# SeunghwanByun/SLAM-RGBD

Measured on AMD Instinct MI355X. Metric: ICP frame-pair aligns/sec @640×480 (1/2/4/8 GPU); SE(3) err vs CPU ref, higher is better.
Workload: dtype fp32

## Files before the change

### slam-rgbd_amd/csrc/icp_api.cpp

```cpp

#include <stdio.h>
#include <stdlib.h>
#include <string.h>

#include <algorithm>
#include <cmath>
#include <vector>

#include "icp_host.h"

using namespace youth_icp;

namespace youth_icp {

thread_local youth::ErrorText g_icp_err;

hipStream_t pick_stream(youth_icp_ctx* c, void* stream)
{
    return stream ? (hipStream_t)stream : c->stream;
}

int bind_device(youth_icp_ctx* c)
{
    HIP_TRY(hipSetDevice(c->device));
// ... 187 lines not shown
        return fail("hipMalloc depth", e);
    if ((e = hipMalloc(&c->d_rec, rec_bytes)) != hipSuccess) return fail("hipMalloc rec", e);
    if ((e = hipMemset(c->d_rec, 0, rec_bytes)) != hipSuccess) return fail("memset rec", e);
    if ((e = hipMalloc(&c->d_T64, MF * 16 * sizeof(double))) != hipSuccess)
        return fail("hipMalloc T64", e);
    if ((e = hipMalloc(&c->d_T32, MF * 12 * sizeof(float))) != hipSuccess)
        return fail("hipMalloc T32", e);
    if ((e = hipMalloc(&c->d_status, MF * sizeof(int32_t))) != hipSuccess)
        return fail("hipMalloc status", e);
    if ((e = hipMalloc(&c->d_Tinit, MF * 16 * sizeof(double))) != hipSuccess)
        return fail("hipMalloc Tinit", e);
    if ((e = hipMalloc(&c->d_neq, MF * kNeq * sizeof(double))) != hipSuccess)
        return fail("hipMalloc neq", e);
    if ((e = hipMalloc(&c->d_Tout, MF * 16 * sizeof(float))) != hipSuccess)
        return fail("hipMalloc Tout", e);
    if ((e = hipMalloc(&c->d_flag, 16)) != hipSuccess) return fail("hipMalloc flag", e);
    if ((e = hipMalloc(&c->d_epoch, MF * sizeof(unsigned))) != hipSuccess)
        return fail("hipMalloc epoch", e);
    if ((e = hipMalloc(&c->d_head, kQWords * 4)) != hipSuccess) return fail("hipMalloc head", e);
    if ((e = hipMemset(c->d_head, 0, kQWords * 4)) != hipSuccess) return fail("memset head", e);
    {
        hipDeviceProp_t prop;
        if ((e = hipGetDeviceProperties(&prop, device)) != hipSuccess)
            return fail("hipGetDeviceProperties", e);
        c->n_cu = prop.multiProcessorCount;
        const char* what = nullptr;
        if ((e = fill_occupancy(c, &what)) != hipSuccess) return fail(what, e);
        const char* np = getenv("YOUTH_ICP_NO_PERSISTENT");
        c->persistent = !(np && *np && *np != '0');
        const char* nif = getenv("YOUTH_ICP_NO_IDENT_FIRST");
        c->ident_first = ident_first_ok(Kd) && !(nif && *nif && *nif != '0');
        const char* ifm = getenv("YOUTH_ICP_IDENT_FIRST");
        c->ident_prep = !(ifm && strcmp(ifm, "icp") == 0);
        const char* pst = getenv("YOUTH_ICP_PREP_STRIP");
        if (pst && atoi(pst) >= 1) c->prep_strip = atoi(pst);
        const char* cth = getenv("YOUTH_ICP_COOP_THREADS");
        if (cth && atoi(cth) == 256) c->coop_threads = 256;
        const char* nc = getenv("YOUTH_ICP_NO_COOP");
        c->coop = !(nc && *nc && *nc != '0');
        const char* cpd = getenv("YOUTH_ICP_COOP_POLL_DELAY");
        if (cpd && atoi(cpd) >= 0) c->coop_poll_delay = atoi(cpd);
        const char* cpx = getenv("YOUTH_ICP_COOP_PX");
        if (cpx && atoi(cpx) >= 1 && atoi(cpx) <= kCoopMaxPx) c->coop_px = atoi(cpx);
        c->coop_px_env = c->coop_px;
        const char* cl = getenv("YOUTH_ICP_COOP_LAUNCH");
        c->coop_launch = !cl ? 0 : strcmp(cl, "runtime") == 0 ? 1 : strcmp(cl, "plain") == 0 ? 2 : 0;
        const char* tcp = getenv("YOUTH_ICP_TRACK_COPY");
        c->trk_copy_compute = tcp && strcmp(tcp, "compute") == 0;
        c->trk_copy_sdma = tcp && (strcmp(tcp, "sdma") == 0 || c->trk_copy_compute);
        const char* pwg = getenv("YOUTH_ICP_PULL_WG");
        c->trk_pull_wg = pwg && atoi(pwg) > 0 ? std::min(atoi(pwg), 1024) : 0;
        const char* plds = getenv("YOUTH_ICP_PULL_LDS");
        if (plds && atoi(plds) >= 0) c->trk_pull_lds = std::min(atoi(plds), 64 << 10);
        const char* pres = getenv("YOUTH_ICP_PULL_RESERVE_CU");
        if (pres && atoi(pres) >= 0) c->trk_pull_reserve = atoi(pres);
        const char* cpt = getenv("YOUTH_ICP_COPY_THREADS");
        if (cpt && atoi(cpt) >= 0) c->trk_copy_helpers = std::min(atoi(cpt), 15);
        const char* cst = getenv("YOUTH_ICP_TEST_COOP_STALL");
        if (cst && atoi(cst) >= 0) {
            c->coop_stall_once = atoi(cst);
            const char* colon = strchr(cst, ':');
            c->coop_stall_left = colon && atoi(colon + 1) > 0 ? atoi(colon + 1) : 1;
            fprintf(stderr, "youth_icp: TEST HOOK YOUTH_ICP_TEST_COOP_STALL=%s active: the first %d "
                            "cooperative launch(es) of this context time out\n",
                    cst, c->coop_stall_left);
        }
        const char* sit = getenv("YOUTH_ICP_TEST_COOP_STALL_ITER");
        if (sit && atoi(sit) >= 0) c->coop_stall_iter = atoi(sit);
// ... 348 lines not shown
```

### slam-rgbd_amd/csrc/icp_device.h

```cpp
#ifndef YOUTH_ICP_DEVICE_H
#define YOUTH_ICP_DEVICE_H

#include <hip/hip_runtime.h>

#include <stdint.h>

#include "youth_icp.h"

namespace {

constexpr int kTileW = 64;
constexpr int kPrepThreads = 512;
#ifndef YOUTH_PREP_TW
#define YOUTH_PREP_TW 128
#endif
#ifndef YOUTH_PREP_TH
#define YOUTH_PREP_TH 24
#endif
constexpr int kPrepTW = YOUTH_PREP_TW;
constexpr int kPrepTH = YOUTH_PREP_TH;
constexpr int kLdsW = kTileW + 2;

constexpr int kRedThreads = 256;
constexpr int kRedStep = kRedThreads * 4;
constexpr int kNeq = YOUTH_NEQ;
constexpr int kPartStride = 30;
constexpr int kPieces = kPartStride / 2;
constexpr int kSumCols = 16;
constexpr int kQHead = 0, kQError = 32, kQSpins = 64, kQWaited = 96, kQHeads = 128;
constexpr int kMaxQueues = 8, kQHeadStride = 32;
constexpr int kQWords = kQHeads + kMaxQueues * kQHeadStride;

typedef float f4v __attribute__((ext_vector_type(4)));
typedef unsigned u4v __attribute__((ext_vector_type(4)));

struct Intr {
    float fx, fy, cx, cy, ds;
};

struct FastK {
    float hfx, lfx, hfy, lfy, hds, lds;
};

__device__ __forceinline__ double join64(unsigned lo, unsigned hi)
{
    return __hiloint2double((int)hi, (int)lo);
}
__device__ __forceinline__ unsigned lo32(double x) { return (unsigned)__double2loint(x); }
__device__ __forceinline__ unsigned hi32(double x) { return (unsigned)__double2hiint(x); }

__device__ __forceinline__ double readlane64(double x, int l)
{
    return join64((unsigned)__builtin_amdgcn_readlane((int)lo32(x), l),
// ... 63 lines not shown
{
    return (len2 >= 0x1p-96f) && (len2 <= 0x1p118f) && norm_comp_ok(cx) && norm_comp_ok(cy) &&
           norm_comp_ok(cz);
}
__device__ __forceinline__ float norm_div(float c, float len, float r)
{
    return copysignf(proj_quot(fabsf(c), len, r), c);
}
__device__ __forceinline__ bool norm_fast_ok_bits(float len2, float cx, float cy, float cz)
{
    constexpr unsigned kLo = 0x0F800000u, kHi = 0x7A800000u, kTiny = 2u * 0x1F800000u - 2u;
    const unsigned tx = (__float_as_uint(cx) << 1) - 2u, ty = (__float_as_uint(cy) << 1) - 2u,
                   tz = (__float_as_uint(cz) << 1) - 2u;
    return (int)((__float_as_uint(len2) - kLo) <= (kHi - kLo)) & (int)(min(min(tx, ty), tz) >= kTiny);
}

template <bool kFast>
__device__ __forceinline__ void backproject(int d, int u, int v, const Intr& K,
                                            const FastK& F, float& x, float& y, float& z)
{
    const float zz = bp_div<kFast>((float)max(d, 0), K.ds, F.hds, F.lds);
    x = bp_div<kFast>(((float)u - K.cx) * zz, K.fx, F.hfx, F.lfx);
    y = bp_div<kFast>(((float)v - K.cy) * zz, K.fy, F.hfy, F.lfy);
    z = zz;
}
template <bool kFast>
__device__ __forceinline__ void backproject_c(int d, float uc, float vc, const Intr& K,
                                              const FastK& F, float& x, float& y, float& z)
{
    const float zz = bp_div<kFast>((float)max(d, 0), K.ds, F.hds, F.lds);
    x = bp_div<kFast>(uc * zz, K.fx, F.hfx, F.lfx);
    y = bp_div<kFast>(vc * zz, K.fy, F.hfy, F.lfy);
    z = zz;
}

__device__ __forceinline__ double dd2(double a, double b, double c, double d)
{
    return fma(a, b, -(c * d));
}
__device__ __forceinline__ double dot3(double a0, double b0, double a1, double b1, double a2,
                                       double b2)
{
    return fma(a2, b2, fma(a1, b1, a0 * b0));
}
__device__ __forceinline__ void adj3(const double* p, double* c)
{
    c[0] = dd2(p[3], p[5], p[4], p[4]);
    c[1] = dd2(p[2], p[4], p[1], p[5]);
    c[2] = dd2(p[1], p[4], p[2], p[3]);
    c[3] = dd2(p[0], p[5], p[2], p[2]);
    c[4] = dd2(p[1], p[2], p[0], p[4]);
    c[5] = dd2(p[0], p[3], p[1], p[1]);
}
__device__ __forceinline__ void symv3(const double* c, const double* v, double* o)
{
    o[0] = dot3(c[0], v[0], c[1], v[1], c[2], v[2]);
    o[1] = dot3(c[1], v[0], c[3], v[1], c[4], v[2]);
    o[2] = dot3(c[2], v[0], c[4], v[1], c[5], v[2]);
}
__device__ __forceinline__ int solve_block6(const double* neq, double xi[6])
{
#pragma unroll
    for (int i = 0; i < 6; ++i) xi[i] = 0.0;
    if (!(neq[28] >= 6.0)) return YOUTH_STATUS_FEW_MATCHES;
    double maxd = 0.0;
    maxd = neq[0] > maxd ? neq[0] : maxd;
// ... 498 lines not shown
```

### slam-rgbd_amd/csrc/icp_host.h

```cpp
#ifndef YOUTH_ICP_HOST_H
#define YOUTH_ICP_HOST_H

#include <hip/hip_runtime.h>

#include <stddef.h>
#include <stdint.h>

#include <memory>
#include <string>
#include <vector>

#include "hip_host.h"
#include "host_copy.h"
#include "icp_device.h"
#include "youth_icp.h"

namespace youth_icp __attribute__((visibility("hidden"))) {

extern thread_local youth::ErrorText g_icp_err;

}

#define HIP_ERR youth_icp::g_icp_err

// ... 9 lines not shown
    int W = 0, H = 0, N = 0;
    size_t P = 0;
    int max_frames = 0;
    Intr K{};
    FastK F{};
    bool fast = false;
    bool centred_exact = true;
    int spec = kSpecSurvey;
    youth_icp_params prm{};
    hipStream_t stream = nullptr;

    int16_t* d_depth = nullptr;
    float4* d_rec = nullptr;
    float* d_xyz = nullptr;
    double* d_T64 = nullptr;
    float* d_T32 = nullptr;
    int32_t* d_status = nullptr;
    double* d_Tinit = nullptr;
    double* d_stats = nullptr;
    int stats_iters = 0;
    double* d_partials = nullptr;
    size_t partials_cap = 0;
    double* d_neq = nullptr;
    int32_t* d_assoc = nullptr;
    float* d_Tout = nullptr;
    unsigned* d_flag = nullptr;
    unsigned* d_arrivals = nullptr;
    unsigned* d_arr_it = nullptr;
    unsigned* d_epoch = nullptr;
    unsigned* d_head = nullptr;
    bool persistent = true;
    bool ident_first = true;
    bool ident_prep = true;
    int prep_strip = 0;
    int last_first_form = 0;
    int reduce = YOUTH_REDUCE_EXACT;
    youth_lanes lanes{};
    bool has_lanes = false;
    bool lanes_mixed = false;
    int icp_blocks_per_cu[4 * kVariants] = {};
    int n_cu = 0;
    bool coop = true;
    int coop_px = 0;
    int coop_px_env = 0;
    int coop_threads = 512;
    int coop_max_pairs = kCoopMaxPairs;
    int coop_launch = 0;
    bool trk_copy_compute = false;
    bool trk_copy_sdma = false;
    int trk_pull_wg = 0;
    int trk_pull_lds = 48 << 10;
    int trk_pull_reserve = 32;
    int trk_copy_helpers = 3;
    size_t trk_copy_min = 1u << 20;
    std::unique_ptr<youth::HostCopyPool> copy_pool;
    bool coop_refuse = false;
    int coop_bpc[2][2 * kVariants][kCoopMaxPx + 1] = {};
    int coop_bpc_tall[2 * kVariants] = {};
    unsigned* d_coop = nullptr;
    int32_t* d_status_out = nullptr;
    int coop_par = 0;
    double* d_coop_part = nullptr;
    int coop_part_cap = 0;
    int coop_part_rows[2] = {0, 0};
    int coop_poll_delay = -1;
    int coop_stall_once = -1;
    int coop_stall_left = 0;
// ... 115 lines not shown
```

### slam-rgbd_amd/csrc/icp_kernels.hip

```cpp

#include <hip/hip_runtime.h>

#include <stdint.h>
#include <stdio.h>
#include <stdlib.h>

#include <algorithm>
#include <cmath>
#include <condition_variable>
#include <mutex>

#include "icp_device.h"
#include "icp_host.h"

namespace {

__global__ void k_verify_fastdiv(Intr K, FastK F, int W, int H, unsigned* bad)
{
    const int d = blockIdx.x * blockDim.x + threadIdx.x + 1;
    if (d > 32767) return;
    const float zi = (float)d / K.ds;
    unsigned nb = (div_fast((float)d, F.hds, F.lds) != zi);
    for (int u = blockIdx.y; u < W; u += gridDim.y) {
        const float n = ((float)u - K.cx) * zi;
// ... 124 lines not shown
    constexpr unsigned kLo = 0x0F800000u, kHi = 0x7A800000u;
    for (unsigned long long b = kLo + tid; b <= kHi; b += stride) {
        const float x = __uint_as_float((unsigned)b);
        b0 += __float_as_uint(sqrt_rn_mid(x)) != __float_as_uint(sqrtf(x));
    }
    for (unsigned long long i = tid; i < n; i += stride) {
        unsigned long long st = seed ^ (i * 0xD1B54A32D192ED03ull);
        const int e0 = (int)(sm64(st) % 131) - 70;
        float c[3];
#pragma unroll
        for (int k = 0; k < 3; ++k) {
            const unsigned long long r = sm64(st);
            const int e = max(e0 - (int)((r >> 32) % 48), -126);
            const unsigned sign = (unsigned)(r >> 63) << 31;
            c[k] = ((r >> 56) & 7) == 0
                       ? __uint_as_float(sign)
                       : __uint_as_float(sign | (unsigned)((e + 127) << 23) |
                                         (unsigned)(r & 0x7FFFFF));
        }
        const float len2 = (c[0] * c[0] + c[1] * c[1]) + c[2] * c[2];
        b1 += norm_fast_ok_bits(len2, c[0], c[1], c[2]) != norm_fast_ok(len2, c[0], c[1], c[2]);
        if (!(len2 > 0.0f) || !norm_fast_ok(len2, c[0], c[1], c[2])) continue;
        ++nf;
        const float len = sqrt_rn_mid(len2), r = proj_recip(len), ref = sqrtf(len2);
#pragma unroll
        for (int k = 0; k < 3; ++k)
            b1 += __float_as_uint(norm_div(c[k], len, r)) != __float_as_uint(c[k] / ref);
    }
    if (b0) atomicAdd(bad + 0, b0);
    if (b1) atomicAdd(bad + 1, b1);
    if (nf) atomicAdd(bad + 2, nf);
}

template <bool kFast, bool kWide, bool kSc1, int kThreads, int kTH, int kTW = kTileW, typename Fn>
__device__ __forceinline__ void prep_tile_with(const int16_t* __restrict__ dep,
                                               float4* __restrict__ R, int W, int H, size_t P,
                                               const Intr& K, const FastK& F,
                                               float* __restrict__ X, int x0, int y0, float* sX,
                                               float* sY, float* sZ, Fn&& per_record)
{
    constexpr int kLH = kTH + 2;
    constexpr int kLW = kTW + 2;
    static_assert(kTW % 64 == 0 && kThreads % kTW == 0, "rows of whole waves");
    static_assert(kTH % (kThreads / kTW) == 0, "tile rows a multiple of the rows per step");
    static_assert(3 * (kTH + 2) * (kTW + 2) * sizeof(float) <= 160 * 1024, "LDS planes fit");
    const int tx = threadIdx.x % kTW;
    const int ty = threadIdx.x / kTW;
    if (kWide) {
        static_assert(2 * kLH <= kThreads, "one edge pixel per thread");
        const bool edge = threadIdx.x < 2 * kLH;
        const int ely = threadIdx.x >> 1, eright = threadIdx.x & 1;
        const int egy = y0 - 1 + ely, egx = eright ? x0 + kTW : x0 - 1;
        const __amdgpu_buffer_rsrc_t rdep = __builtin_amdgcn_make_buffer_rsrc(
            const_cast<int16_t*>(dep), (short)0, W * H * (int)sizeof(int16_t), 0x00020000);
        const bool ein = edge & ((unsigned)egy < (unsigned)H) & ((unsigned)egx < (unsigned)W);
        unsigned short dedge =
            __builtin_amdgcn_raw_buffer_load_b16(rdep, ein ? (egy * W + egx) * 2 : W * H * 2, 0, 0);
        constexpr int kWords = kTW / 4;
        constexpr int kIt = (kLH * kWords + kThreads - 1) / kThreads;
        short4 wd[kIt];
#pragma unroll
        for (int it = 0; it < kIt; ++it) {
            const int e = threadIdx.x + it * kThreads;
            const int ly = e / kWords;
            const int gy = y0 - 1 + ly;
            const int c = x0 + 4 * (e - ly * kWords);
            const bool inside = (e < kLH * kWords) & ((unsigned)gy < (unsigned)H) & (c < W);
            wd[it] = __builtin_bit_cast(
                short4, __builtin_amdgcn_raw_buffer_load_b64(rdep, inside ? (gy * W + c) * 2 : W * H * 2, 0, 0));
        }
#pragma unroll
        for (int it = 0; it < kIt; ++it) {
// ... 39 lines not shown
            const int ly = e / kLW;
            const int lx = e - ly * kLW;
            const int gx = x0 - 1 + lx, gy = y0 - 1 + ly;
            float x = 0.0f, y = 0.0f, z = 0.0f;
            if (gx >= 0 && gx < W && gy >= 0 && gy < H)
                backproject<kFast>(dep[(size_t)gy * W + gx], gx, gy, K, F, x, y, z);
            sX[ly * kLW + lx] = x;
            sY[ly * kLW + lx] = y;
            sZ[ly * kLW + lx] = z;
        }
    }
    __syncthreads();

    const __amdgpu_buffer_rsrc_t rrec =
        __builtin_amdgcn_make_buffer_rsrc(R, (short)0, (int)(P * sizeof(float4)), 0x00020000);
    const int tyw = __builtin_amdgcn_readfirstlane(ty);
#pragma unroll
    for (int k = 0; k < kTH / (kThreads / kTW); ++k) {
        const int row = tyw + (kThreads / kTW) * k;
        const int gx = x0 + tx, gy = y0 + row;
        if (gx >= W || gy >= H) continue;
        const size_t i = (size_t)gy * W + gx;
        const int ly = row + 1, lx = tx + 1;
        const int o = ly * kLW + lx;
        const float px = sX[o], py = sY[o], pz = sZ[o];
        if (X) {
            X[i] = px;
            X[P + i] = py;
            X[2 * P + i] = pz;
        }
        const bool inner = (gx > 0) & (gy > 0) & (gx < W - 1) & (gy < H - 1);
        const float zl = sZ[o - 1], zr = sZ[o + 1];
        const float zu = sZ[o - kLW], zd = sZ[o + kLW];
        const unsigned zmin = min(min(min(__float_as_uint(pz), __float_as_uint(zl)),
                                      min(__float_as_uint(zr), __float_as_uint(zu))),
                                  __float_as_uint(zd));
        const float ax = sX[o + 1] - sX[o - 1];
        const float ay = sY[o + 1] - sY[o - 1];
        const float az = zr - zl;
        const float bx = sX[o + kLW] - sX[o - kLW];
        const float by = sY[o + kLW] - sY[o - kLW];
        const float bz = zd - zu;
        const float cx = ay * bz - az * by;
        const float cy = az * bx - ax * bz;
        const float cz = ax * by - ay * bx;
        const float len2 = (cx * cx + cy * cy) + cz * cz;
        const bool has_n = inner & (zmin != 0u) & (len2 > 0.0f);
        const float len = sqrt_rn_mid(len2);
        const float r = proj_recip(len);
        float nx = norm_div(cx, len, r);
        float ny = norm_div(cy, len, r);
        float nz = norm_div(cz, len, r);
        if (__builtin_expect(has_n & !norm_fast_ok_bits(len2, cx, cy, cz), 0)) {
            const float l = sqrtf(len2);
            nx = cx / l;
            ny = cy / l;
            nz = cz / l;
        }
        if (((nx * px + ny * py) + nz * pz) > 0.0f) {
            nx = -nx;
            ny = -ny;
            nz = -nz;
        }
        if (!has_n) nx = ny = nz = 0.0f;
        const float4 rec = make_float4(has_n ? pz : 0.0f, nx, ny, nz);
        if (kSc1) {
            __builtin_amdgcn_raw_buffer_store_b128(__builtin_bit_cast(u4v, rec), rrec,
                                                   (int)(i * sizeof(float4)), 0, 16);
        } else {
            __builtin_amdgcn_raw_buffer_store_b128(__builtin_bit_cast(u4v, rec), rrec,
                                                   (int)(i * sizeof(float4)), 0, 2);
        }
        per_record(k, px, py, pz, rec);
    }
}

template <bool kFast, bool kWide, bool kSc1, int kThreads, int kTH, int kTW = kTileW>
__device__ __forceinline__ void prep_tile(const int16_t* __restrict__ dep, float4* __restrict__ R,
                                          int W, int H, size_t P, const Intr& K, const FastK& F,
                                          float* __restrict__ X, int x0, int y0, float* sX,
                                          float* sY, float* sZ)
{
    prep_tile_with<kFast, kWide, kSc1, kThreads, kTH, kTW>(
        dep, R, W, H, P, K, F, X, x0, y0, sX, sY, sZ,
        [](int, float, float, float, const float4&) __attribute__((always_inline)) {});
}

struct InitArgs {
    const double* T_init;
    int n;
    double* T64;
    float* T32;
    int32_t* status;
    unsigned* epoch;
    unsigned* arrivals;
    int iters;
    unsigned* head_err;
};

__device__ __forceinline__ void init_pairs(const InitArgs& ia, int tx, int ty, int f, int n_frames)
{
    if (tx != 0 || ty != 0) return;
    if (f == 0 && threadIdx.x < kMaxQueues && ia.head_err) {
        if (threadIdx.x == 0) {
            ia.head_err[kQHead] = 0u;
            ia.head_err[kQError] = 0u;
            ia.head_err[kQSpins] = 0u;
            ia.head_err[kQWaited] = 0u;
        }
        ia.head_err[kQHeads + kQHeadStride * threadIdx.x] = 0u;
    }
    const int t = threadIdx.x;
    for (int p = f; p < ia.n; p += n_frames) {
        if (t < 16) {
            const double v = ia.T_init ? ia.T_init[(size_t)p * 16 + t] : ((t % 5) == 0 ? 1.0 : 0.0);
            ia.T64[(size_t)p * 16 + t] = v;
            if (t < 12) ia.T32[(size_t)p * 12 + t] = (float)v;
        } else if (t == 16) {
// ... 593 lines not shown
                    st_u64_sc1(is.T64 + (size_t)p * 16 + lane,
                               (unsigned long long)__double_as_longlong(sh_T64[lane]));
                    st_u32_sc1(is.T32 + (size_t)p * 12 + lane, __float_as_uint(sh_T32n[lane]));
                }
                if (k == is.iters - 1 && is.T_out && lane < 16)
                    is.T_out[(size_t)p * 16 + lane] =
                        lane < 12 ? sh_T32n[lane] : (lane == 15 ? 1.0f : 0.0f);
                asm volatile("s_waitcnt vmcnt(0)" ::: "memory");
                if (lane == 0) st_u32_sc1(is.epoch + p, (unsigned)(k + 1));
            }
        }
        if (threadIdx.x == 0) sh_item = icp_claim(is, sh_next, total, per_iter, sh_T);
        __syncthreads();
    }
}

struct IdentArgs {
    const int16_t* dsrc;
    PairMap pm;
    int n_pairs, iters;
    float thr2;
    double* partials;
    double* T64;
    float* T32;
    int32_t* status;
    double* stats;
    unsigned* epoch;
    unsigned* arr_it;
    unsigned* arrivals;
    float* T_out;
    unsigned* head_err;
};

template <int kSp, bool kFast, bool kWide>
__global__ __launch_bounds__(kPrepThreads) void k_prep_ident(const int16_t* __restrict__ depth,
                                                            int out0, int W, int H, size_t P,
                                                            Intr K, FastK F,
                                                            float4* __restrict__ recs, IdentArgs ia,
                                                            int tiles_x, int tiles_y, int strip)
{
    static_assert(!sp_lane32(kSp), "exact sums only");
    constexpr int kRows = kPrepThreads / kPrepTW;
    constexpr int kSteps = kPrepTH / kRows;
    constexpr int kWaves = kPrepThreads / 64;
    __shared__ float sX[(kPrepTH + 2) * (kPrepTW + 2)];
    __shared__ float sY[(kPrepTH + 2) * (kPrepTW + 2)];
    __shared__ float sZ[(kPrepTH + 2) * (kPrepTW + 2)];
    static_assert(sizeof(sX) >= kWaves * kNeq * sizeof(double), "the waves' sums fit a plane");
    static_assert(sizeof(sY) >= (32 + 16) * sizeof(double) + 12 * sizeof(float), "solve scratch");
    const int per = tiles_x * tiles_y;
    const int strips = (per + strip - 1) / strip;
    const int f = (int)blockIdx.x / strips;
    const int sidx = (int)blockIdx.x - f * strips;
    if (blockIdx.x == 0 && threadIdx.x < kMaxQueues && ia.head_err) {
        if (threadIdx.x == 0) {
            ia.head_err[kQHead] = 0u;
            ia.head_err[kQError] = 0u;
            ia.head_err[kQSpins] = 0u;
            ia.head_err[kQWaited] = 0u;
        }
        ia.head_err[kQHeads + kQHeadStride * threadIdx.x] = 0u;
    }
    const int N = W * H;
    const int p = out0 + f - ia.pm.tgt0;
    const bool paired = (unsigned)p < (unsigned)ia.n_pairs;
    const __amdgpu_buffer_rsrc_t rsrc = __builtin_amdgcn_make_buffer_rsrc(
        const_cast<int16_t*>(ia.dsrc + (size_t)(ia.pm.src0 + (paired ? p : 0)) * N), (short)0,
        N * (int)sizeof(int16_t), 0x00020000);
    const int tx = threadIdx.x % kPrepTW;
    const int tyw = __builtin_amdgcn_readfirstlane((int)threadIdx.x / kPrepTW);
    const int lane = threadIdx.x & 63;
    const int wave = threadIdx.x >> 6;
    double acc[kNeq];
#pragma unroll
    for (int q = 0; q < kNeq; ++q) acc[q] = 0.0;
    int cnt = 0;

    const int t0 = sidx * strip, t1 = min(t0 + strip, per);
    for (int r = t0; r < t1; ++r) {
        const int tyi = r / tiles_x;
        const int x0 = (r - tyi * tiles_x) * kPrepTW, y0 = tyi * kPrepTH;
        int sd[kSteps];
#pragma unroll
        for (int k = 0; k < kSteps; ++k) {
            const int gx = x0 + tx, gy = y0 + tyw + kRows * k;
            const bool in = paired & (gx < W) & (gy < H);
            sd[k] = (short)__builtin_amdgcn_raw_buffer_load_b16(rsrc, in ? (gy * W + gx) * 2 : N * 2,
                                                                0, 0);
        }
        if (r > t0) __syncthreads();
        prep_tile_with<kFast, kWide, false, kPrepThreads, kPrepTH, kPrepTW>(
            depth + (size_t)f * N, recs + (size_t)(out0 + f) * P, W, H, P, K, F, nullptr, x0, y0, sX,
            sY, sZ,
            [&](int k, float px, float py, float pz, const float4& rec)
                __attribute__((always_inline)) {
                    if (!paired) return;
                    float sx, sy, sz;
                    backproject<kFast>(sd[k], x0 + tx, y0 + tyw + kRows * k, K, F, sx, sy, sz);
                    const f4v t = {rec.x, rec.y, rec.z, rec.w};
                    const LaneMask okm = ident_accumulate_xy<kSp, true>(sx, sy, sz, px, py, t,
                                                                        ia.thr2, acc);
                    cnt += lane_in(okm) ? 1 : 0;
                });
    }
    if (!paired) return;
    acc[28] = (double)cnt;
    double tot;
    wave_reduce_scatter<kNeq>(acc, lane, tot);
    __syncthreads();
    double(*red)[kNeq] = reinterpret_cast<double(*)[kNeq]>(sX);
    if (!(lane & 1) && (lane >> 1) < kNeq) red[wave][lane >> 1] = tot;
    __syncthreads();
    if (threadIdx.x >= 64) return;
    double s = 0.0;
    if (lane < kNeq) {
        double w[kWaves];
#pragma unroll
        for (int q = 0; q < kWaves; ++q) w[q] = red[q][lane];
        s = tree_sum<kWaves>(w);
    }
    PoseState ps{};
    ps.arrivals = ia.arrivals;
    if (!handoff_publish<kNeq>(ia.partials + ((size_t)p * strips + sidx) * kPartStride, ps, p, strips,
                               lane, s))
        return;
    double neq[kNeq];
    handoff_sum<kNeq, kPartStride>(ia.partials, p, strips, lane, neq);
    double* sh_neq = reinterpret_cast<double*>(sY);
    double* sh_T64 = sh_neq + 32;
    float* sh_T32 = reinterpret_cast<float*>(sh_T64 + 16);
    if (lane == 0) {
#pragma unroll
        for (int q = 0; q < kNeq; ++q) sh_neq[q] = neq[q];
    }
    if (lane < 16) sh_T64[lane] = (lane % 5) == 0 ? 1.0 : 0.0;
    if (lane < 12) sh_T32[lane] = (lane % 5) == 0 ? 1.0f : 0.0f;
    const int st = solve_update_wave_call(sh_neq, sh_T64, sh_T32, lane);
    if (lane < 16) ia.T64[(size_t)p * 16 + lane] = sh_T64[lane];
    if (lane < 12) ia.T32[(size_t)p * 12 + lane] = sh_T32[lane];
    if (ia.iters == 1 && ia.T_out && lane < 16)
        ia.T_out[(size_t)p * 16 + lane] = lane < 12 ? sh_T32[lane] : (lane == 15 ? 1.0f : 0.0f);
    for (int k = lane; k < ia.iters; k += 64) ia.arr_it[(size_t)p * ia.iters + k] = 0u;
    if (lane == 0) {
        ia.status[p] = st;
        ia.epoch[p] = 1u;
        ia.arrivals[p] = 0u;
        if (ia.stats) {
            ia.stats[(size_t)p * ia.iters * 2 + 0] = neq[28];
            ia.stats[(size_t)p * ia.iters * 2 + 1] = neq[27];
        }
    }
}


struct CoopState {
    const double* T_init;
    double* T64;
    float* T32;
    int32_t* status;
    double* stats;
    float* T_out;
    unsigned* set;
    unsigned* set_next;
// ... 548 lines not shown
}

static int launch_prep_with(youth_icp_ctx* c, hipStream_t s, const int16_t* depth, int n_frames,
                            int out0, bool want_xyz, const InitArgs* init)
{
    if (n_frames <= 0) return YOUTH_OK;
    if (want_xyz) {
        int rc = ensure_xyz(c);
        if (rc) return rc;
    }
    const int tiles_x = (c->W + kPrepTW - 1) / kPrepTW, tiles_y = (c->H + kPrepTH - 1) / kPrepTH;
    const long long rows = (long long)tiles_y * n_frames;
    const long long blocks = (long long)tiles_x * (c->prep_xcd_map == 2 ? (rows + 7) / 8 * 8 : rows);
    if (blocks > 0x7fffffffLL) return g_icp_err.set(YOUTH_EINVAL, "launch_prep: %lld tiles", blocks);
    EventPair ep{};
    int rc = ev_begin(c, s, &ep, 2);
    if (rc) return rc;
    float* xyz = want_xyz ? c->d_xyz : nullptr;
    const bool wide = (c->W % 4 == 0) && (reinterpret_cast<uintptr_t>(depth) % 8 == 0);
    auto kern = c->fast ? (wide ? k_prep<true, true> : k_prep<true, false>)
                        : (wide ? k_prep<false, true> : k_prep<false, false>);
    const InitArgs ia = init ? *init : InitArgs{};
    hipLaunchKernelGGL(kern, dim3((unsigned)blocks), dim3(kPrepThreads), 0, s, depth, out0, c->W,
                       c->H, c->P, c->K, c->F, c->d_rec, xyz, ia, tiles_x, tiles_y, n_frames,
                       c->prep_xcd_map);
    HIP_TRY(hipGetLastError());
    return ev_end(c, s, &ep);
}

typedef void (*PrepIdentKernel)(const int16_t*, int, int, int, size_t, Intr, FastK, float4*,
                                IdentArgs, int, int, int);
static PrepIdentKernel prep_ident_kernel(int idx)
{
    static const PrepIdentKernel tab[8] = {
        k_prep_ident<0, false, false>, k_prep_ident<0, false, true>, k_prep_ident<0, true, false>,
        k_prep_ident<0, true, true>,   k_prep_ident<1, false, false>, k_prep_ident<1, false, true>,
        k_prep_ident<1, true, false>,  k_prep_ident<1, true, true>};
    return tab[idx & 7];
}

static int launch_prep_ident(youth_icp_ctx* c, hipStream_t s, const PrepJob* job,
                             const int16_t* dsrc, PairMap pm, int n_pairs, int iters, float thr2,
                             int nb, float* d_T_out)
{
    const int tiles_x = (c->W + kPrepTW - 1) / kPrepTW, tiles_y = (c->H + kPrepTH - 1) / kPrepTH;
    const int per = tiles_x * tiles_y;
    int strip = c->prep_strip;
    if (strip <= 0) {
        strip = (int)std::min<long long>(25, (long long)per * job->n / (8LL * c->n_cu));
        strip = std::max(strip, 5);
    }
    strip = std::min(strip, per);
    const int strips = (per + strip - 1) / strip;
    const long long blocks = (long long)strips * job->n;
    if (blocks > 0x7fffffffLL) return g_icp_err.set(YOUTH_EINVAL, "launch_prep: %lld strips", blocks);
    int rc = ensure_partials(c, (size_t)std::max(nb, strips) * n_pairs * kPartStride);
    if (rc) return rc;
    EventPair ep{};
    rc = ev_begin(c, s, &ep, 2);
    if (rc) return rc;
    const bool wide = (c->W % 4 == 0) && (reinterpret_cast<uintptr_t>(job->depth) % 8 == 0);
    const IdentArgs ia{dsrc,      pm,        n_pairs,     iters,      thr2,
                       c->d_partials, c->d_T64, c->d_T32,  c->d_status, c->d_stats,
                       c->d_epoch, c->d_arr_it, c->d_arrivals, d_T_out,  c->d_head};
    auto kern = prep_ident_kernel(c->spec * 4 + (c->fast ? 2 : 0) + (wide ? 1 : 0));
    hipLaunchKernelGGL(kern, dim3((unsigned)blocks), dim3(kPrepThreads), 0, s, job->depth, job->out0,
                       c->W, c->H, c->P, c->K, c->F, c->d_rec, ia, tiles_x, tiles_y, strip);
    HIP_TRY(hipGetLastError());
    return ev_end(c, s, &ep);
}

int launch_prep(youth_icp_ctx* c, hipStream_t s, const int16_t* depth, int n_frames, int out0,
                bool want_xyz)
{
    return launch_prep_with(c, s, depth, n_frames, out0, want_xyz, nullptr);
}

template <int kSp, bool kAssoc, bool kFast, bool kAligned, bool kFuse>
static void launch_reduce_t(youth_icp_ctx* c, hipStream_t s, dim3 grid, const int16_t* dsrc,
                            PairMap pm, float thr2, int chunk, const PoseState& ps)
{
    hipLaunchKernelGGL((k_reduce<kSp, kAssoc, kFast, kAligned, kFuse>), grid, dim3(kRedThreads), 0,
                       s, dsrc, c->d_rec, c->P, pm, c->W, c->H, c->K, c->F, thr2, chunk,
                       c->d_partials, kAssoc ? c->d_assoc : (int32_t*)nullptr, ps);
}

template <int kSp>
static void launch_reduce_sel(youth_icp_ctx* c, hipStream_t s, dim3 grid, const int16_t* dsrc,
                              PairMap pm, float thr2, int chunk, const PoseState& ps, int sel)
{
    switch (sel) {
    case 0: launch_reduce_t<kSp, false, false, false, false>(c, s, grid, dsrc, pm, thr2, chunk, ps); break;
    case 1: launch_reduce_t<kSp, false, false, true, false>(c, s, grid, dsrc, pm, thr2, chunk, ps); break;
    case 2: launch_reduce_t<kSp, false, true, false, false>(c, s, grid, dsrc, pm, thr2, chunk, ps); break;
    case 3: launch_reduce_t<kSp, false, true, true, false>(c, s, grid, dsrc, pm, thr2, chunk, ps); break;
    case 4: launch_reduce_t<kSp, false, false, false, true>(c, s, grid, dsrc, pm, thr2, chunk, ps); break;
    case 5: launch_reduce_t<kSp, false, false, true, true>(c, s, grid, dsrc, pm, thr2, chunk, ps); break;
    case 6: launch_reduce_t<kSp, false, true, false, true>(c, s, grid, dsrc, pm, thr2, chunk, ps); break;
    case 7: launch_reduce_t<kSp, false, true, true, true>(c, s, grid, dsrc, pm, thr2, chunk, ps); break;
    case 8: launch_reduce_t<kSp, true, false, false, false>(c, s, grid, dsrc, pm, thr2, chunk, ps); break;
// ... 487 lines not shown
```

Measured before the change: 89930.

## Rewrite fused prep+identity kernel as single-wave column bands with DPP neighbours

The fused prep/identity-ICP kernel moves from 512-thread 2D LDS tiles to one 64-lane wave per 64-column, band-of-rows unit. Each lane walks down its column and keeps the up, centre and down points in registers. Left and right neighbours come from DPP lane shifts, and the wave-edge lanes load the halo columns. This removes the LDS staging, the __syncthreads barriers and the cross-wave reduction, and it software-pipelines the row loads. In exchange there are many more small blocks, and therefore more partials in the handoff sum. The wide/aligned specialisation is also dropped.

```diff
diff --git a/slam-rgbd_amd/csrc/icp_api.cpp b/slam-rgbd_amd/csrc/icp_api.cpp
--- a/slam-rgbd_amd/csrc/icp_api.cpp
+++ b/slam-rgbd_amd/csrc/icp_api.cpp
@@ -243,8 +243,8 @@
         c->ident_first = ident_first_ok(Kd) && !(nif && *nif && *nif != '0');
         const char* ifm = getenv("YOUTH_ICP_IDENT_FIRST");
         c->ident_prep = !(ifm && strcmp(ifm, "icp") == 0);
-        const char* pst = getenv("YOUTH_ICP_PREP_STRIP");
-        if (pst && atoi(pst) >= 1) c->prep_strip = atoi(pst);
+        const char* pbd = getenv("YOUTH_ICP_PREP_BAND");
+        if (pbd && atoi(pbd) >= 1) c->prep_band = atoi(pbd);
         const char* cth = getenv("YOUTH_ICP_COOP_THREADS");
         if (cth && atoi(cth) == 256) c->coop_threads = 256;
         const char* nc = getenv("YOUTH_ICP_NO_COOP");
diff --git a/slam-rgbd_amd/csrc/icp_device.h b/slam-rgbd_amd/csrc/icp_device.h
--- a/slam-rgbd_amd/csrc/icp_device.h
+++ b/slam-rgbd_amd/csrc/icp_device.h
@@ -19,6 +19,8 @@
 #endif
 constexpr int kPrepTW = YOUTH_PREP_TW;
 constexpr int kPrepTH = YOUTH_PREP_TH;
+constexpr int kPrepColW = 64;
+constexpr int kPrepBand = 96;
 constexpr int kLdsW = kTileW + 2;
 
 constexpr int kRedThreads = 256;
@@ -148,6 +150,45 @@
     x = bp_div<kFast>(uc * zz, K.fx, F.hfx, F.lfx);
     y = bp_div<kFast>(vc * zz, K.fy, F.hfy, F.lfy);
     z = zz;
+}
+
+__device__ __forceinline__ float4 prep_record(float px, float py, float pz, float lx, float ly,
+                                              float lz, float rx, float ry, float rz, float ux,
+                                              float uy, float uz, float dx, float dy, float dz,
+                                              bool inner)
+{
+    const unsigned zmin = min(min(min(__float_as_uint(pz), __float_as_uint(lz)),
+                                  min(__float_as_uint(rz), __float_as_uint(uz))),
+                              __float_as_uint(dz));
+    const float ax = rx - lx;
+    const float ay = ry - ly;
+    const float az = rz - lz;
+    const float bx = dx - ux;
+    const float by = dy - uy;
+    const float bz = dz - uz;
+    const float cx = ay * bz - az * by;
+    const float cy = az * bx - ax * bz;
+    const float cz = ax * by - ay * bx;
+    const float len2 = (cx * cx + cy * cy) + cz * cz;
+    const bool has_n = inner & (zmin != 0u) & (len2 > 0.0f);
+    const float len = sqrt_rn_mid(len2);
+    const float r = proj_recip(len);
+    float nx = norm_div(cx, len, r);
+    float ny = norm_div(cy, len, r);
+    float nz = norm_div(cz, len, r);
+    if (__builtin_expect(has_n & !norm_fast_ok_bits(len2, cx, cy, cz), 0)) {
+        const float l = sqrtf(len2);
+        nx = cx / l;
+        ny = cy / l;
+        nz = cz / l;
+    }
+    if (((nx * px + ny * py) + nz * pz) > 0.0f) {
+        nx = -nx;
+        ny = -ny;
+        nz = -nz;
+    }
+    if (!has_n) nx = ny = nz = 0.0f;
+    return make_float4(has_n ? pz : 0.0f, nx, ny, nz);
 }
 
 __device__ __forceinline__ double dd2(double a, double b, double c, double d)
diff --git a/slam-rgbd_amd/csrc/icp_host.h b/slam-rgbd_amd/csrc/icp_host.h
--- a/slam-rgbd_amd/csrc/icp_host.h
+++ b/slam-rgbd_amd/csrc/icp_host.h
@@ -65,7 +65,7 @@
     bool persistent = true;
     bool ident_first = true;
     bool ident_prep = true;
-    int prep_strip = 0;
+    int prep_band = 0;
     int last_first_form = 0;
     int reduce = YOUTH_REDUCE_EXACT;
     youth_lanes lanes{};
diff --git a/slam-rgbd_amd/csrc/icp_kernels.hip b/slam-rgbd_amd/csrc/icp_kernels.hip
--- a/slam-rgbd_amd/csrc/icp_kernels.hip
+++ b/slam-rgbd_amd/csrc/icp_kernels.hip
@@ -180,12 +180,11 @@
     if (nf) atomicAdd(bad + 2, nf);
 }
 
-template <bool kFast, bool kWide, bool kSc1, int kThreads, int kTH, int kTW = kTileW, typename Fn>
-__device__ __forceinline__ void prep_tile_with(const int16_t* __restrict__ dep,
-                                               float4* __restrict__ R, int W, int H, size_t P,
-                                               const Intr& K, const FastK& F,
-                                               float* __restrict__ X, int x0, int y0, float* sX,
-                                               float* sY, float* sZ, Fn&& per_record)
+template <bool kFast, bool kWide, bool kSc1, int kThreads, int kTH, int kTW = kTileW>
+__device__ __forceinline__ void prep_tile(const int16_t* __restrict__ dep, float4* __restrict__ R,
+                                          int W, int H, size_t P, const Intr& K, const FastK& F,
+                                          float* __restrict__ X, int x0, int y0, float* sX,
+                                          float* sY, float* sZ)
 {
     constexpr int kLH = kTH + 2;
     constexpr int kLW = kTW + 2;
@@ -291,38 +290,11 @@
         const bool inner = (gx > 0) & (gy > 0) & (gx < W - 1) & (gy < H - 1);
         const float zl = sZ[o - 1], zr = sZ[o + 1];
         const float zu = sZ[o - kLW], zd = sZ[o + kLW];
-        const unsigned zmin = min(min(min(__float_as_uint(pz), __float_as_uint(zl)),
-                                      min(__float_as_uint(zr), __float_as_uint(zu))),
-                                  __float_as_uint(zd));
-        const float ax = sX[o + 1] - sX[o - 1];
-        const float ay = sY[o + 1] - sY[o - 1];
-        const float az = zr - zl;
-        const float bx = sX[o + kLW] - sX[o - kLW];
-        const float by = sY[o + kLW] - sY[o - kLW];
-        const float bz = zd - zu;
-        const float cx = ay * bz - az * by;
-        const float cy = az * bx - ax * bz;
-        const float cz = ax * by - ay * bx;
-        const float len2 = (cx * cx + cy * cy) + cz * cz;
-        const bool has_n = inner & (zmin != 0u) & (len2 > 0.0f);
-        const float len = sqrt_rn_mid(len2);
-        const float r = proj_recip(len);
-        float nx = norm_div(cx, len, r);
-        float ny = norm_div(cy, len, r);
-        float nz = norm_div(cz, len, r);
-        if (__builtin_expect(has_n & !norm_fast_ok_bits(len2, cx, cy, cz), 0)) {
-            const float l = sqrtf(len2);
-            nx = cx / l;
-            ny = cy / l;
-            nz = cz / l;
-        }
-        if (((nx * px + ny * py) + nz * pz) > 0.0f) {
-            nx = -nx;
-            ny = -ny;
-            nz = -nz;
-        }
-        if (!has_n) nx = ny = nz = 0.0f;
-        const float4 rec = make_float4(has_n ? pz : 0.0f, nx, ny, nz);
+        const float xr = sX[o + 1], xl = sX[o - 1];
+        const float yr = sY[o + 1], yl = sY[o - 1];
+        const float xd = sX[o + kLW], xu = sX[o - kLW];
+        const float yd = sY[o + kLW], yu = sY[o - kLW];
+        const float4 rec = prep_record(px, py, pz, xl, yl, zl, xr, yr, zr, xu, yu, zu, xd, yd, zd, inner);
         if (kSc1) {
             __builtin_amdgcn_raw_buffer_store_b128(__builtin_bit_cast(u4v, rec), rrec,
                                                    (int)(i * sizeof(float4)), 0, 16);
@@ -330,19 +302,7 @@
             __builtin_amdgcn_raw_buffer_store_b128(__builtin_bit_cast(u4v, rec), rrec,
                                                    (int)(i * sizeof(float4)), 0, 2);
         }
-        per_record(k, px, py, pz, rec);
-    }
-}
-
-template <bool kFast, bool kWide, bool kSc1, int kThreads, int kTH, int kTW = kTileW>
-__device__ __forceinline__ void prep_tile(const int16_t* __restrict__ dep, float4* __restrict__ R,
-                                          int W, int H, size_t P, const Intr& K, const FastK& F,
-                                          float* __restrict__ X, int x0, int y0, float* sX,
-                                          float* sY, float* sZ)
-{
-    prep_tile_with<kFast, kWide, kSc1, kThreads, kTH, kTW>(
-        dep, R, W, H, P, K, F, X, x0, y0, sX, sY, sZ,
-        [](int, float, float, float, const float4&) __attribute__((always_inline)) {});
+    }
 }
 
 struct InitArgs {
@@ -1002,103 +962,133 @@
     unsigned* head_err;
 };
 
-template <int kSp, bool kFast, bool kWide>
-__global__ __launch_bounds__(kPrepThreads) void k_prep_ident(const int16_t* __restrict__ depth,
-                                                            int out0, int W, int H, size_t P,
-                                                            Intr K, FastK F,
-                                                            float4* __restrict__ recs, IdentArgs ia,
-                                                            int tiles_x, int tiles_y, int strip)
+__device__ __forceinline__ float from_left(float v, float edge)
+{
+    return __int_as_float(__builtin_amdgcn_update_dpp(__float_as_int(edge), __float_as_int(v),
+                                                      0x138, 0xf, 0xf, false));
+}
+__device__ __forceinline__ float from_right(float v, float edge)
+{
+    return __int_as_float(__builtin_amdgcn_update_dpp(__float_as_int(edge), __float_as_int(v),
+                                                      0x130, 0xf, 0xf, false));
+}
+
+struct PrepRowIn {
+    unsigned t;
+    unsigned e;
+    unsigned s;
+};
+
+template <int kSp, bool kFast>
+__global__ __launch_bounds__(kPrepColW) void k_prep_ident(const int16_t* depth, int out0, int W,
+                                                         int H, size_t P, Intr K, FastK F,
+                                                         float4* recs, IdentArgs ia, int blocks_x,
+                                                         int bands, int band)
 {
     static_assert(!sp_lane32(kSp), "exact sums only");
-    constexpr int kRows = kPrepThreads / kPrepTW;
-    constexpr int kSteps = kPrepTH / kRows;
-    constexpr int kWaves = kPrepThreads / 64;
-    __shared__ float sX[(kPrepTH + 2) * (kPrepTW + 2)];
-    __shared__ float sY[(kPrepTH + 2) * (kPrepTW + 2)];
-    __shared__ float sZ[(kPrepTH + 2) * (kPrepTW + 2)];
-    static_assert(sizeof(sX) >= kWaves * kNeq * sizeof(double), "the waves' sums fit a plane");
-    static_assert(sizeof(sY) >= (32 + 16) * sizeof(double) + 12 * sizeof(float), "solve scratch");
-    const int per = tiles_x * tiles_y;
-    const int strips = (per + strip - 1) / strip;
-    const int f = (int)blockIdx.x / strips;
-    const int sidx = (int)blockIdx.x - f * strips;
-    if (blockIdx.x == 0 && threadIdx.x < kMaxQueues && ia.head_err) {
-        if (threadIdx.x == 0) {
+    static_assert(kPrepColW == 64 && kMaxQueues <= kPrepColW, "one wave per unit");
+    __shared__ double sh_neq[32 + 16];
+    __shared__ float sh_T32[12];
+    const int lane = threadIdx.x;
+    const int per = blocks_x * bands;
+    const int f = (int)blockIdx.x / per;
+    const int unit = (int)blockIdx.x - f * per;
+    const int bi = unit / blocks_x;
+    const int x0 = (unit - bi * blocks_x) * kPrepColW;
+    const int y0 = bi * band, y1 = min(y0 + band, H);
+    if (blockIdx.x == 0 && lane < kMaxQueues && ia.head_err) {
+        if (lane == 0) {
             ia.head_err[kQHead] = 0u;
             ia.head_err[kQError] = 0u;
             ia.head_err[kQSpins] = 0u;
             ia.head_err[kQWaited] = 0u;
         }
-        ia.head_err[kQHeads + kQHeadStride * threadIdx.x] = 0u;
+        ia.head_err[kQHeads + kQHeadStride * lane] = 0u;
     }
     const int N = W * H;
     const int p = out0 + f - ia.pm.tgt0;
     const bool paired = (unsigned)p < (unsigned)ia.n_pairs;
+    const __amdgpu_buffer_rsrc_t rdep = __builtin_amdgcn_make_buffer_rsrc(
+        const_cast<int16_t*>(depth + (size_t)f * N), (short)0, N * (int)sizeof(int16_t), 0x00020000);
     const __amdgpu_buffer_rsrc_t rsrc = __builtin_amdgcn_make_buffer_rsrc(
         const_cast<int16_t*>(ia.dsrc + (size_t)(ia.pm.src0 + (paired ? p : 0)) * N), (short)0,
-        N * (int)sizeof(int16_t), 0x00020000);
-    const int tx = threadIdx.x % kPrepTW;
-    const int tyw = __builtin_amdgcn_readfirstlane((int)threadIdx.x / kPrepTW);
-    const int lane = threadIdx.x & 63;
-    const int wave = threadIdx.x >> 6;
+        paired ? N * (int)sizeof(int16_t) : 0, 0x00020000);
+    const __amdgpu_buffer_rsrc_t rrec = __builtin_amdgcn_make_buffer_rsrc(
+        recs + (size_t)(out0 + f) * P, (short)0, (int)(P * sizeof(float4)), 0x00020000);
+    const int oob = N * 2;
+    const int gx = x0 + lane;
+    const int col2 = gx < W ? gx * 2 : oob;
+    const int ex = lane == 0 ? x0 - 1 : x0 + kPrepColW;
+    const bool eload = ((lane == 0) | (lane == kPrepColW - 1)) & ((unsigned)ex < (unsigned)W);
+    const int ecol2 = eload ? ex * 2 : oob;
+    const int rcol = gx < W ? gx * (int)sizeof(float4) : (int)(P * sizeof(float4));
+
+    auto row2 = [&](int y, bool want) { return (want & ((unsigned)y < (unsigned)H)) ? y * W * 2 : oob; };
+    auto load_tgt = [&](int off) {
+        return (unsigned)__builtin_amdgcn_raw_buffer_load_b16(rdep, off, 0, 0);
+    };
+    auto load_row = [&](int y) {
+        const int rd = row2(y + 1, y < y1), rc = row2(y, y < y1);
+        PrepRowIn r;
+        r.t = load_tgt(col2 + rd);
+        r.e = load_tgt(ecol2 + rc);
+        r.s = (unsigned)__builtin_amdgcn_raw_buffer_load_b16(rsrc, col2 + rc, 0, 0);
+        return r;
+    };
+
     double acc[kNeq];
 #pragma unroll
     for (int q = 0; q < kNeq; ++q) acc[q] = 0.0;
     int cnt = 0;
 
-    const int t0 = sidx * strip, t1 = min(t0 + strip, per);
-    for (int r = t0; r < t1; ++r) {
-        const int tyi = r / tiles_x;
-        const int x0 = (r - tyi * tiles_x) * kPrepTW, y0 = tyi * kPrepTH;
-        int sd[kSteps];
-#pragma unroll
-        for (int k = 0; k < kSteps; ++k) {
-            const int gx = x0 + tx, gy = y0 + tyw + kRows * k;
-            const bool in = paired & (gx < W) & (gy < H);
-            sd[k] = (short)__builtin_amdgcn_raw_buffer_load_b16(rsrc, in ? (gy * W + gx) * 2 : N * 2,
-                                                                0, 0);
-        }
-        if (r > t0) __syncthreads();
-        prep_tile_with<kFast, kWide, false, kPrepThreads, kPrepTH, kPrepTW>(
-            depth + (size_t)f * N, recs + (size_t)(out0 + f) * P, W, H, P, K, F, nullptr, x0, y0, sX,
-            sY, sZ,
-            [&](int k, float px, float py, float pz, const float4& rec)
-                __attribute__((always_inline)) {
-                    if (!paired) return;
-                    float sx, sy, sz;
-                    backproject<kFast>(sd[k], x0 + tx, y0 + tyw + kRows * k, K, F, sx, sy, sz);
-                    const f4v t = {rec.x, rec.y, rec.z, rec.w};
-                    const LaneMask okm = ident_accumulate_xy<kSp, true>(sx, sy, sz, px, py, t,
-                                                                        ia.thr2, acc);
-                    cnt += lane_in(okm) ? 1 : 0;
-                });
-    }
+    const int t_up = (short)load_tgt(col2 + row2(y0 - 1, true));
+    const int t_c = (short)load_tgt(col2 + row2(y0, true));
+    PrepRowIn in0 = load_row(y0), in1 = load_row(y0 + 1);
+    float ux, uy, uz, cx, cy, cz;
+    backproject<kFast>(t_up, gx, y0 - 1, K, F, ux, uy, uz);
+    backproject<kFast>(t_c, gx, y0, K, F, cx, cy, cz);
+    auto row = [&](int y, PrepRowIn& in) __attribute__((always_inline)) {
+        int dt = (short)in.t, de = (short)in.e, dsr = (short)in.s;
+        asm volatile("" : "+v"(dt), "+v"(de), "+v"(dsr));
+        in = load_row(y + 2);
+        float dx, dy, dz, ox, oy, oz;
+        backproject<kFast>(dt, gx, y + 1, K, F, dx, dy, dz);
+        backproject<kFast>(de, ex, y, K, F, ox, oy, oz);
+        const bool inner = (gx > 0) & (y > 0) & (gx < W - 1) & (y < H - 1);
+        const float4 rec =
+            prep_record(cx, cy, cz, from_left(cx, ox), from_left(cy, oy), from_left(cz, oz),
+                        from_right(cx, ox), from_right(cy, oy), from_right(cz, oz), ux, uy, uz, dx,
+                        dy, dz, inner);
+        __builtin_amdgcn_raw_buffer_store_b128(__builtin_bit_cast(u4v, rec), rrec,
+                                               rcol + y * W * (int)sizeof(float4), 0, 2);
+        float sx, sy, sz;
+        backproject<kFast>(dsr, gx, y, K, F, sx, sy, sz);
+        const f4v t = {rec.x, rec.y, rec.z, rec.w};
+        const LaneMask okm = ident_accumulate_xy<kSp, true>(sx, sy, sz, cx, cy, t, ia.thr2, acc);
+        cnt += lane_in(okm) ? 1 : 0;
+        ux = cx, uy = cy, uz = cz;
+        cx = dx, cy = dy, cz = dz;
+    };
+    __builtin_amdgcn_s_waitcnt(0x0F70);
+    int y = y0;
+    for (; y + 1 < y1; y += 2) {
+        row(y, in0);
+        row(y + 1, in1);
+    }
+    if (y < y1) row(y, in0);
     if (!paired) return;
     acc[28] = (double)cnt;
     double tot;
     wave_reduce_scatter<kNeq>(acc, lane, tot);
-    __syncthreads();
-    double(*red)[kNeq] = reinterpret_cast<double(*)[kNeq]>(sX);
-    if (!(lane & 1) && (lane >> 1) < kNeq) red[wave][lane >> 1] = tot;
-    __syncthreads();
-    if (threadIdx.x >= 64) return;
-    double s = 0.0;
-    if (lane < kNeq) {
-        double w[kWaves];
-#pragma unroll
-        for (int q = 0; q < kWaves; ++q) w[q] = red[q][lane];
-        s = tree_sum<kWaves>(w);
-    }
+    const double s = __shfl(tot, (2 * lane) & 63, 64);
     PoseState ps{};
     ps.arrivals = ia.arrivals;
-    if (!handoff_publish<kNeq>(ia.partials + ((size_t)p * strips + sidx) * kPartStride, ps, p, strips,
-                               lane, s))
+    if (!handoff_publish<kNeq>(ia.partials + ((size_t)p * per + unit) * kPartStride, ps, p, per, lane,
+                               s))
         return;
     double neq[kNeq];
-    handoff_sum<kNeq, kPartStride>(ia.partials, p, strips, lane, neq);
-    double* sh_neq = reinterpret_cast<double*>(sY);
+    handoff_sum<kNeq, kPartStride>(ia.partials, p, per, lane, neq);
     double* sh_T64 = sh_neq + 32;
-    float* sh_T32 = reinterpret_cast<float*>(sh_T64 + 16);
     if (lane == 0) {
 #pragma unroll
         for (int q = 0; q < kNeq; ++q) sh_neq[q] = neq[q];
@@ -1713,40 +1703,37 @@
                                 IdentArgs, int, int, int);
 static PrepIdentKernel prep_ident_kernel(int idx)
 {
-    static const PrepIdentKernel tab[8] = {
-        k_prep_ident<0, false, false>, k_prep_ident<0, false, true>, k_prep_ident<0, true, false>,
-        k_prep_ident<0, true, true>,   k_prep_ident<1, false, false>, k_prep_ident<1, false, true>,
-        k_prep_ident<1, true, false>,  k_prep_ident<1, true, true>};
-    return tab[idx & 7];
+    static const PrepIdentKernel tab[4] = {k_prep_ident<0, false>, k_prep_ident<0, true>,
+                                           k_prep_ident<1, false>, k_prep_ident<1, true>};
+    return tab[idx & 3];
 }
 
 static int launch_prep_ident(youth_icp_ctx* c, hipStream_t s, const PrepJob* job,
                              const int16_t* dsrc, PairMap pm, int n_pairs, int iters, float thr2,
                              int nb, float* d_T_out)
 {
-    const int tiles_x = (c->W + kPrepTW - 1) / kPrepTW, tiles_y = (c->H + kPrepTH - 1) / kPrepTH;
-    const int per = tiles_x * tiles_y;
-    int strip = c->prep_strip;
-    if (strip <= 0) {
-        strip = (int)std::min<long long>(25, (long long)per * job->n / (8LL * c->n_cu));
-        strip = std::max(strip, 5);
-    }
-    strip = std::min(strip, per);
-    const int strips = (per + strip - 1) / strip;
-    const long long blocks = (long long)strips * job->n;
-    if (blocks > 0x7fffffffLL) return g_icp_err.set(YOUTH_EINVAL, "launch_prep: %lld strips", blocks);
-    int rc = ensure_partials(c, (size_t)std::max(nb, strips) * n_pairs * kPartStride);
+    const int blocks_x = (c->W + kPrepColW - 1) / kPrepColW;
+    int band = c->prep_band;
+    if (band <= 0) {
+        const long long rows = (long long)c->H * blocks_x * job->n / (4LL * c->n_cu);
+        band = (int)std::max<long long>(std::min<long long>(kPrepBand, rows), 24);
+    }
+    band = std::min(band, c->H);
+    const int bands = (c->H + band - 1) / band;
+    const int per = blocks_x * bands;
+    const long long blocks = (long long)per * job->n;
+    if (blocks > 0x7fffffffLL) return g_icp_err.set(YOUTH_EINVAL, "launch_prep: %lld units", blocks);
+    int rc = ensure_partials(c, (size_t)std::max(nb, per) * n_pairs * kPartStride);
     if (rc) return rc;
     EventPair ep{};
     rc = ev_begin(c, s, &ep, 2);
     if (rc) return rc;
-    const bool wide = (c->W % 4 == 0) && (reinterpret_cast<uintptr_t>(job->depth) % 8 == 0);
     const IdentArgs ia{dsrc,      pm,        n_pairs,     iters,      thr2,
                        c->d_partials, c->d_T64, c->d_T32,  c->d_status, c->d_stats,
                        c->d_epoch, c->d_arr_it, c->d_arrivals, d_T_out,  c->d_head};
-    auto kern = prep_ident_kernel(c->spec * 4 + (c->fast ? 2 : 0) + (wide ? 1 : 0));
-    hipLaunchKernelGGL(kern, dim3((unsigned)blocks), dim3(kPrepThreads), 0, s, job->depth, job->out0,
-                       c->W, c->H, c->P, c->K, c->F, c->d_rec, ia, tiles_x, tiles_y, strip);
+    auto kern = prep_ident_kernel(c->spec * 2 + (c->fast ? 1 : 0));
+    hipLaunchKernelGGL(kern, dim3((unsigned)blocks), dim3(kPrepColW), 0, s, job->depth, job->out0,
+                       c->W, c->H, c->P, c->K, c->F, c->d_rec, ia, blocks_x, bands, band);
     HIP_TRY(hipGetLastError());
     return ev_end(c, s, &ep);
 }
```

New measurement: 91520, median of 6. +1.8%, better.
